# Li-Qingyun/RSCoTr

Measured on AMD Instinct MI355X. Metric: images/sec MTL train step (Swin-T 512^2, bs=2/GPU), higher is better.
Workload: dtype f32 (large products as three fp16 MFMAs on two-plane power-of-two-scaled splits of the fp32 operands, fp32 accumulate: fp32-FMA-class error; six bf16 MFMAs on three-plane splits where an operand has no range word)

## Files before the change

rscotr_amd/csrc/swin_attn.hip:

```cpp
#include "common.h"
#include "rscotr.h"

namespace rscotr {

constexpr int WS = 7, WN = 49, HD = 32, TBL = 169;
constexpr int WATTN_PBIAS = 172, WATTN_PROW = WATTN_PBIAS + 3 * HD;

struct WinGeom {
  int H, W, Hp, Wp, nWw, nW, C, heads, shift;
};

struct TokPos {
  bool pad;
  long tok;
  int label;
};

__device__ __forceinline__ TokPos win_token(const WinGeom& g, int wy, int wx, int t) {
  TokPos r;
  const int ys = wy * WS + t / WS, xs = wx * WS + t % WS;
  int yo = ys + g.shift, xo = xs + g.shift;
  if (yo >= g.Hp) yo -= g.Hp;
  if (xo >= g.Wp) xo -= g.Wp;
  r.pad = (yo >= g.H) || (xo >= g.W);
  r.tok = (long)yo * g.W + xo;
  const int ry = ys < g.Hp - WS ? 0 : (ys < g.Hp - g.shift ? 1 : 2);
  const int rx = xs < g.Wp - WS ? 0 : (xs < g.Wp - g.shift ? 1 : 2);
  r.label = ry * 3 + rx;
  return r;
}

constexpr int LDT = HD + 1;
constexpr int NPD = WN + 1;
constexpr int LDP = NPD + 1;

typedef float f32x16 __attribute__((ext_vector_type(16)));

struct TileRegs {
  float4 v[(WN * (HD / 4) + 63) / 64];
};

__device__ __forceinline__ void tile_load(TileRegs& r, const float* __restrict__ src_tok0, long tok_stride,
                                          const float* __restrict__ pad_vals, const int* sTok, int lane) {
#pragma unroll
  for (int i = 0; i < 7; ++i) {
    const int idx = lane + i * 64;
    r.v[i] = make_float4(0.f, 0.f, 0.f, 0.f);
    if (idx < WN * (HD / 4)) {
      const int t = idx >> 3, c4 = idx & 7;
      const int tok = sTok[t];
      if (tok >= 0) r.v[i] = *reinterpret_cast<const float4*>(src_tok0 + (long)tok * tok_stride + c4 * 4);
      else if (pad_vals) r.v[i] = *reinterpret_cast<const float4*>(pad_vals + c4 * 4);
    }
  }
}

__device__ __forceinline__ void tile_store(const TileRegs& r, float* dst, float scale, int lane) {
#pragma unroll
  for (int i = 0; i < 7; ++i) {
    const int idx = lane + i * 64;
    if (idx < WN * (HD / 4)) {
      float* d = dst + (idx >> 3) * LDT + (idx & 7) * 4;
      d[0] = r.v[i].x * scale; d[1] = r.v[i].y * scale; d[2] = r.v[i].z * scale; d[3] = r.v[i].w * scale;
    }
  }
}

__device__ __forceinline__ void zero16(f32x16& a) {
#pragma unroll
  for (int r = 0; r < 16; ++r) a[r] = 0.f;
}

__device__ __forceinline__ int crow(int r, int lane) { return (r & 3) + 8 * (r >> 2) + 4 * (lane >> 5); }

__device__ __forceinline__ float half_sum(float v) {
#pragma unroll
  for (int o = 16; o > 0; o >>= 1) v += __shfl_xor(v, o, 64);
  return v;
}

__device__ __forceinline__ void mma_rr1(f32x16& acc, const float* A, const float* B, int mi, int ni, int lane) {
  const int fr = lane & 31, fk = lane >> 5;
  const float* a = A + min(mi * 32 + fr, WN - 1) * LDT + fk;
  const float* b = B + min(ni * 32 + fr, WN - 1) * LDT + fk;
#pragma unroll
  for (int kk = 0; kk < HD; kk += 2) acc = __builtin_amdgcn_mfma_f32_32x32x2f32(a[kk], b[kk], acc, 0, 0, 0);
}

__device__ __forceinline__ void mma_pt1(f32x16& acc, const float* SP, const float* T, int mi, int lane) {
  const int fr = lane & 31, fk = lane >> 5;
  const float* a = SP + min(mi * 32 + fr, WN) * LDP + fk;
#pragma unroll 5
  for (int kk = 0; kk < NPD; kk += 2)
    acc = __builtin_amdgcn_mfma_f32_32x32x2f32(a[kk], T[min(kk + fk, WN - 1) * LDT + fr], acc, 0, 0, 0);
}

__device__ __forceinline__ void mma_ptT1(f32x16& acc, const float* SP, const float* T, int mi, int lane) {
  const int fr = lane & 31, fk = lane >> 5;
  const int j = min(mi * 32 + fr, WN);
#pragma unroll 5
  for (int kk = 0; kk < NPD; kk += 2)
    acc = __builtin_amdgcn_mfma_f32_32x32x2f32(SP[(kk + fk) * LDP + j], T[min(kk + fk, WN - 1) * LDT + fr], acc, 0, 0, 0);
}

__device__ __forceinline__ void store_scores1(const f32x16& acc, float* sP, const float* sT, const int* sLab, int shift,
                                              int mi, int ni, int lane) {
  const int fr = lane & 31;
  const int j = ni * 32 + fr, jc = min(j, WN - 1);
  const int jb = (6 - jc / WS) * 13 + (6 - jc % WS), jl = sLab[jc];
#pragma unroll
  for (int r = 0; r < 16; ++r) {
    const int i = mi * 32 + crow(r, lane);
    if (i >= WN || j >= WN) continue;
    const int ti = (i / WS) * 13 + i % WS;
    sP[i * LDP + j] = acc[r] + sT[ti + jb] + ((shift > 0 && jl != sLab[i]) ? -100.0f : 0.f);
  }
}

__device__ __forceinline__ void softmax_rows4(float* sP, int tid) {
  const int row = tid >> 2, q = tid & 3;
  float* rowp = sP + min(row, WN - 1) * LDP;
  float v[13];
  float m = -3.0e38f;
#pragma unroll
  for (int u = 0; u < 13; ++u) {
    const int j = q + 4 * u;
    v[u] = j < WN ? rowp[j] : -3.0e38f;
    m = fmaxf(m, v[u]);
  }
  m = fmaxf(m, __shfl_xor(m, 1, 64));
  m = fmaxf(m, __shfl_xor(m, 2, 64));
  float sum = 0.f;
#pragma unroll
  for (int u = 0; u < 13; ++u) {
    v[u] = (q + 4 * u < WN) ? __expf(v[u] - m) : 0.f;
    sum += v[u];
  }
  sum += __shfl_xor(sum, 1, 64);
  sum += __shfl_xor(sum, 2, 64);
  const float inv = 1.f / sum;
  if (row < WN) {
#pragma unroll
    for (int u = 0; u < 13; ++u)
      if (q + 4 * u < WN) rowp[q + 4 * u] = v[u] * inv;
  }
}

__device__ __forceinline__ void stage_item_tiles(float* sQ, float* sK, float* sV, float* sG, const float* base,
                                                 const float* __restrict__ qkv_b, const float* dout_b, const WinGeom& g,
                                                 int head, const int* sTok, float scale, int w, int lane) {
  if (w == 3 && !dout_b) return;
  const float* src = w == 3 ? dout_b : base + w * g.C;
  const long tstride = w == 3 ? g.C : 3 * g.C;
  const float* padv = (w == 3 || !qkv_b) ? nullptr : qkv_b + w * g.C + head * HD;
  float* dst = w == 0 ? sQ : (w == 1 ? sK : (w == 2 ? sV : sG));
  TileRegs r;
  tile_load(r, src, tstride, padv, sTok, lane);
  tile_store(r, dst, w == 0 ? scale : 1.f, lane);
}

__global__ __launch_bounds__(256) void swin_wattn_fwd_mfma4_kernel(const float* __restrict__ qkv,
                                                                   const float* __restrict__ qkv_b,
                                                                   const float* __restrict__ table,
                                                                   float* __restrict__ out, WinGeom g, int B,
                                                                   unsigned* __restrict__ amax_out) {
  __shared__ float sQ[WN * LDT], sK[WN * LDT], sV[WN * LDT];
  __shared__ float sP[NPD * LDP];
  __shared__ float sT[TBL];
  __shared__ int sLab[WN], sTok[WN];
  float amx = 0.f;
  const int tid = threadIdx.x, lane = tid & 63, w = tid >> 6;
  const int head = blockIdx.x % g.heads;
  const int stride = gridDim.x / g.heads;
  const float scale = 0.17677669529663687f;
  const long L = (long)g.H * g.W;
  for (int t = tid; t < TBL; t += 256) sT[t] = table[t * g.heads + head];
  for (int t = tid; t < NPD * LDP; t += 256) sP[t] = 0.f;
  for (int bw = blockIdx.x / g.heads; bw < B * g.nW; bw += stride) {
    const int b = bw / g.nW, win = bw % g.nW, wy = win / g.nWw, wx = win % g.nWw;
    __syncthreads();
    if (tid < WN) {
      const TokPos me = win_token(g, wy, wx, tid);
      sLab[tid] = me.label;
      sTok[tid] = me.pad ? -1 : (int)me.tok;
    }
    __syncthreads();
    stage_item_tiles(sQ, sK, sV, nullptr, qkv + (long)b * L * 3 * g.C + head * HD, qkv_b, nullptr, g, head, sTok, scale, w, lane);
    __syncthreads();
    {
      f32x16 a;
      zero16(a);
      mma_rr1(a, sQ, sK, w >> 1, w & 1, lane);
      store_scores1(a, sP, sT, sLab, g.shift, w >> 1, w & 1, lane);
    }
    __syncthreads();
    softmax_rows4(sP, tid);
    __syncthreads();
    if (w < 2) {
      f32x16 o;
      zero16(o);
      mma_pt1(o, sP, sV, w, lane);
#pragma unroll
      for (int r = 0; r < 16; ++r) {
        const int i = w * 32 + crow(r, lane);
        if (i < WN) {
          const int tok = sTok[i];
          if (tok >= 0) { out[((long)b * L + tok) * g.C + head * HD + (lane & 31)] = o[r]; amx = fmaxf(amx, fabsf(o[r])); }
        }
      }
    }
  }
  amax_commit(amax_out, amx);
}

__device__ __forceinline__ void swin_wattn_bwd_mfma4_body(const float* __restrict__ qkv,
                                                                   const float* __restrict__ qkv_b,
                                                                   const float* __restrict__ table,
                                                                   const float* __restrict__ dout,
                                                                   const float* __restrict__ outp,
                                                                   float* __restrict__ dqkv, float* __restrict__ part,
                                                                   const WinGeom& g, int B, unsigned* __restrict__ amax_out) {
  __shared__ float sQ[WN * LDT], sK[WN * LDT], sV[WN * LDT], sG[WN * LDT];
  __shared__ float sP[NPD * LDP];
  __shared__ float sT[TBL];
  __shared__ float sBw[4][3 * HD];
  float amx = 0.f;
  __shared__ float sDelta[64];
  __shared__ int sLab[WN], sTok[WN];
  const int tid = threadIdx.x, lane = tid & 63, w = tid >> 6, fr = lane & 31;
  const int head = blockIdx.x % g.heads;
  const int stride = gridDim.x / g.heads;
  const float scale = 0.17677669529663687f;
  const long L = (long)g.H * g.W;
  for (int t = tid; t < TBL; t += 256) sT[t] = table[t * g.heads + head];
  for (int t = tid; t < NPD * LDP; t += 256) sP[t] = 0.f;
  float dT = 0.f;
  float accB[3] = {0.f, 0.f, 0.f};
  const int tdy = tid / 13 - 6, tdx = tid % 13 - 6;
  const int iy0 = max(0, tdy), iy1 = min(6, 6 + tdy), ix0 = max(0, tdx), ix1 = min(6, 6 + tdx);
  for (int bw = blockIdx.x / g.heads; bw < B * g.nW; bw += stride) {
    const int b = bw / g.nW, win = bw % g.nW, wy = win / g.nWw, wx = win % g.nWw;
    __syncthreads();
    if (tid < WN) {
      const TokPos me = win_token(g, wy, wx, tid);
      sLab[tid] = me.label;
      sTok[tid] = me.pad ? -1 : (int)me.tok;
    }
    __syncthreads();
    float4 o_a = make_float4(0.f, 0.f, 0.f, 0.f), o_b = o_a;
    if (outp && (tid >> 2) < WN) {
      const int tok = sTok[tid >> 2];
      if (tok >= 0) {
        const float4* o4 = reinterpret_cast<const float4*>(outp + ((long)b * L + tok) * g.C + head * HD + (tid & 3) * 8);
        o_a = o4[0];
        o_b = o4[1];
      }
    }
    stage_item_tiles(sQ, sK, sV, sG, qkv + (long)b * L * 3 * g.C + head * HD, qkv_b, dout + (long)b * L * g.C + head * HD, g,
                     head, sTok, scale, w, lane);
    __syncthreads();
    float* dq_base = dqkv + (long)b * L * 3 * g.C + head * HD;
    if (outp) {
      const float* gq = sG + min(tid >> 2, WN - 1) * LDT + (tid & 3) * 8;
      float d = ((o_a.x * gq[0] + o_a.y * gq[1]) + (o_a.z * gq[2] + o_a.w * gq[3])) +
                ((o_b.x * gq[4] + o_b.y * gq[5]) + (o_b.z * gq[6] + o_b.w * gq[7]));
      d += __shfl_xor(d, 1, 64);
      d += __shfl_xor(d, 2, 64);
      if ((tid & 3) == 0) sDelta[tid >> 2] = d;
    }
    {
      f32x16 a;
      zero16(a);
      mma_rr1(a, sQ, sK, w >> 1, w & 1, lane);
      store_scores1(a, sP, sT, sLab, g.shift, w >> 1, w & 1, lane);
    }
    __syncthreads();
    softmax_rows4(sP, tid);
    __syncthreads();
    f32x16 dp[2];
    if (w < 2) {
      zero16(dp[0]); zero16(dp[1]);
      mma_rr1(dp[0], sG, sV, w, 0, lane);
      mma_rr1(dp[1], sG, sV, w, 1, lane);
    } else {
      f32x16 dv;
      zero16(dv);
      mma_ptT1(dv, sP, sG, w - 2, lane);
#pragma unroll
      for (int r = 0; r < 16; ++r) {
        const int j = (w - 2) * 32 + crow(r, lane);
        if (j < WN) {
          const int tok = sTok[j];
          if (tok >= 0) { dq_base[(long)tok * 3 * g.C + 2 * g.C + fr] = dv[r]; amx = fmaxf(amx, fabsf(dv[r])); }
          else accB[2] += dv[r];
        }
      }
    }
    __syncthreads();
    if (w < 2) {
#pragma unroll
      for (int r = 0; r < 16; ++r) {
        const int i = w * 32 + crow(r, lane);
        const bool iv = i < WN;
        const int j0 = fr, j1 = 32 + fr;
        const float p0 = iv ? sP[i * LDP + j0] : 0.f;
        const float p1 = (iv && j1 < WN) ? sP[i * LDP + j1] : 0.f;
        const float delta = outp ? sDelta[min(i, 63)] : half_sum(p0 * dp[0][r] + p1 * dp[1][r]);
        if (iv) {
          sP[i * LDP + j0] = p0 * (dp[0][r] - delta);
          if (j1 < WN) sP[i * LDP + j1] = p1 * (dp[1][r] - delta);
        }
      }
    }
    __syncthreads();
    if (w < 2) {
      f32x16 dq;
      zero16(dq);
      mma_pt1(dq, sP, sK, w, lane);
#pragma unroll
      for (int r = 0; r < 16; ++r) {
        const int i = w * 32 + crow(r, lane);
        if (i < WN) {
          const int tok = sTok[i];
          if (tok >= 0) { dq_base[(long)tok * 3 * g.C + fr] = dq[r] * scale; amx = fmaxf(amx, fabsf(dq[r] * scale)); }
          else accB[0] += dq[r] * scale;
        }
      }
    } else {
      f32x16 dk;
      zero16(dk);
      mma_ptT1(dk, sP, sQ, w - 2, lane);
#pragma unroll
      for (int r = 0; r < 16; ++r) {
        const int j = (w - 2) * 32 + crow(r, lane);
        if (j < WN) {
          const int tok = sTok[j];
          if (tok >= 0) { dq_base[(long)tok * 3 * g.C + g.C + fr] = dk[r]; amx = fmaxf(amx, fabsf(dk[r])); }
          else accB[1] += dk[r];
        }
      }
    }
    if (tid < TBL) {
      float acc7 = 0.f;
#pragma unroll 1
      for (int iy = iy0; iy <= iy1; ++iy) {
        float v[WS];
#pragma unroll
        for (int ix = 0; ix < WS; ++ix) {
          const bool ok = ix >= ix0 && ix <= ix1;
          v[ix] = ok ? sP[(iy * WS + ix) * LDP + (iy - tdy) * WS + (ix - tdx)] : 0.f;
        }
        acc7 += ((v[0] + v[1]) + (v[2] + v[3])) + ((v[4] + v[5]) + v[6]);
      }
      dT += acc7;
    }
  }
#pragma unroll
  for (int k = 0; k < 3; ++k) {
    const float other = __shfl_xor(accB[k], 32, 64);
    if (lane < 32) sBw[w][k * HD + fr] = accB[k] + other;
  }
  __syncthreads();
  float* prow = part + (long)blockIdx.x * WATTN_PROW;
  if (tid < TBL) prow[tid] = dT;
  if (tid < 3 * HD) prow[WATTN_PBIAS + tid] = ((sBw[0][tid] + sBw[1][tid]) + sBw[2][tid]) + sBw[3][tid];
  amax_commit(amax_out, amx);
}

template <int OCC>
__global__ __launch_bounds__(256) __attribute__((amdgpu_waves_per_eu(OCC, OCC))) void swin_wattn_bwd_mfma4_kernel(
    const float* __restrict__ qkv, const float* __restrict__ qkv_b, const float* __restrict__ table,
    const float* __restrict__ dout, const float* __restrict__ outp, float* __restrict__ dqkv, float* __restrict__ part,
    WinGeom g, int B, unsigned* __restrict__ amax_out) {
  swin_wattn_bwd_mfma4_body(qkv, qkv_b, table, dout, outp, dqkv, part, g, B, amax_out);
}

static int wattn_geom(const char* fn, WinGeom* g, int B, int H, int W, int C, int heads, int ws, int shift) {
  if (B < 0 || H <= 0 || W <= 0 || C <= 0 || heads <= 0)
    return fail(RSCOTR_E_SHAPE, "%s: bad shape B=%d H=%d W=%d C=%d heads=%d", fn, B, H, W, C, heads);
  if (ws != WS) return fail(RSCOTR_E_SHAPE, "%s: window size %d (only 7 is built)", fn, ws);
  if (C != heads * HD) return fail(RSCOTR_E_SHAPE, "%s: C=%d must be heads*32 (heads=%d)", fn, C, heads);
  if (shift < 0 || shift >= WS) return fail(RSCOTR_E_SHAPE, "%s: shift %d outside [0,7)", fn, shift);
  g->H = H; g->W = W; g->C = C; g->heads = heads; g->shift = shift;
  g->Hp = (H + WS - 1) / WS * WS;
  g->Wp = (W + WS - 1) / WS * WS;
  g->nWw = g->Wp / WS;
  g->nW = (g->Hp / WS) * g->nWw;
  return RSCOTR_OK;
}

static int wattn_grid(const WinGeom& g, int B, int per_cu) {
  const long items = (long)B * g.nW;
  long per_head = std::min<long>(items, std::max<long>(1, (256L * per_cu) / g.heads));
  return (int)(per_head * g.heads);
}

}

using namespace rscotr;

extern "C" int rscotr_swin_wattn_fwd(const float* qkv, const float* qkv_bias, const float* bias_table,
                                     float* out, int B, int H, int W, int C, int heads, int ws, int shift,
                                     uint32_t* amax_out, void* stream) {
  WinGeom g;
  if (int e = wattn_geom("rscotr_swin_wattn_fwd", &g, B, H, W, C, heads, ws, shift)) return e;
  if (B == 0) return RSCOTR_OK;
  if (!qkv || !bias_table || !out) return fail(RSCOTR_E_ARG, "rscotr_swin_wattn_fwd: null pointer");
  if (!aligned16(qkv) || !aligned16(out) || (qkv_bias && !aligned16(qkv_bias)))
    return fail(RSCOTR_E_ALIGN, "rscotr_swin_wattn_fwd: pointers must be 16-byte aligned");
  const double items = (double)B * ((H + ws - 1) / ws) * ((W + ws - 1) / ws) * heads;
  ProfScope prof(PROF_MFMA, items * 4.0 * 49 * 49 * 32, (hipStream_t)stream, "rscotr::swin_wattn_fwd_kernel");
  swin_wattn_fwd_mfma4_kernel<<<wattn_grid(g, B, 4), 256, 0, (hipStream_t)stream>>>(qkv, qkv_bias, bias_table, out, g, B, amax_out);
  return check_launch("rscotr_swin_wattn_fwd");
}

static int wattn_bwd_grid(const WinGeom& g, int B) { return wattn_grid(g, B, 4); }

namespace rscotr {
__global__ __launch_bounds__(256) void wattn_param_fold_kernel(const float* __restrict__ part, float* __restrict__ dtable,
                                                               float* __restrict__ dqkv_b, int heads, int C, int rows) {
  __shared__ float red[3][64];
  const int lane = threadIdx.x & 63, w = threadIdx.x >> 6;
  const int col = blockIdx.x * 64 + lane, head = blockIdx.y;
  float a = 0.f;
  if (col < WATTN_PROW) {
#pragma unroll 8
    for (int r = w; r < rows; r += 4) a += part[((long)r * heads + head) * WATTN_PROW + col];
  }
  if (w > 0) red[w - 1][lane] = a;
  __syncthreads();
  if (w != 0 || col >= WATTN_PROW) return;
  a += red[0][lane];
  a += red[1][lane];
  a += red[2][lane];
  if (col < TBL) {
    if (dtable) dtable[col * heads + head] += a;
  } else if (col >= WATTN_PBIAS && dqkv_b) {
    const int t = col - WATTN_PBIAS;
    dqkv_b[(t / HD) * C + head * HD + (t % HD)] += a;
  }
}

__global__ __launch_bounds__(256) void wattn_param_flush_kernel(const int64_t* __restrict__ table, int n) {
  __shared__ float red[3][64];
  int e = 0;
  while (e + 1 < n && (int)table[(long)(e + 1) * 16 + 6] <= (int)blockIdx.y) ++e;
  const int64_t* t = table + (long)e * 16;
  const float* part = reinterpret_cast<const float*>(t[0]);
  float* dtable = reinterpret_cast<float*>(t[1]);
  float* dqkv_b = reinterpret_cast<float*>(t[2]);
  const int heads = (int)t[3], C = (int)t[4], rows = (int)t[5], head = (int)blockIdx.y - (int)t[6];
  const int lane = threadIdx.x & 63, w = threadIdx.x >> 6;
  const int col = blockIdx.x * 64 + lane;
  float a = 0.f;
  if (col < WATTN_PROW) {
#pragma unroll 8
    for (int r = w; r < rows; r += 4) a += part[((long)r * heads + head) * WATTN_PROW + col];
  }
  if (w > 0) red[w - 1][lane] = a;
  __syncthreads();
  if (w != 0 || col >= WATTN_PROW) return;
  a += red[0][lane];
  a += red[1][lane];
  a += red[2][lane];
  if (col < TBL) {
    if (dtable) dtable[col * heads + head] += a;
  } else if (col >= WATTN_PBIAS && dqkv_b) {
    const int c = col - WATTN_PBIAS;
    dqkv_b[(c / HD) * C + head * HD + (c % HD)] += a;
  }
}
}

extern "C" int rscotr_swin_wattn_flush(const int64_t* table, int n, int total_heads, void* stream) {
  if (n < 0 || total_heads < 0) return fail(RSCOTR_E_SHAPE, "rscotr_swin_wattn_flush: negative count");
  if (n == 0 || total_heads == 0) return RSCOTR_OK;
  if (!table) return fail(RSCOTR_E_ARG, "rscotr_swin_wattn_flush: null table");
  wattn_param_flush_kernel<<<dim3((WATTN_PROW + 63) / 64, (unsigned)total_heads), 256, 0, (hipStream_t)stream>>>(table, n);
  return check_launch("rscotr_swin_wattn_flush");
}

extern "C" int64_t rscotr_swin_wattn_bwd_workspace(int B, int H, int W, int C, int heads) {
  WinGeom g;
  if (B <= 0 || wattn_geom("rscotr_swin_wattn_bwd_workspace", &g, B, H, W, C, heads, WS, 0)) return 0;
  return (int64_t)wattn_bwd_grid(g, B) * WATTN_PROW * 4;
}

extern "C" int rscotr_swin_wattn_bwd(const float* qkv, const float* qkv_bias, const float* bias_table,
                                     const float* dout, float* dqkv, float* dqkv_bias, float* dbias_table,
                                     int B, int H, int W, int C, int heads, int ws, int shift, const float* out,
                                     float* workspace, int64_t workspace_bytes, uint32_t* amax_out, void* stream) {
  WinGeom g;
  if (int e = wattn_geom("rscotr_swin_wattn_bwd", &g, B, H, W, C, heads, ws, shift)) return e;
  if (B == 0) return RSCOTR_OK;
  if (!qkv || !bias_table || !dout || !dqkv) return fail(RSCOTR_E_ARG, "rscotr_swin_wattn_bwd: null pointer");
  if (!aligned16(qkv) || !aligned16(dout) || !aligned16(dqkv) || (qkv_bias && !aligned16(qkv_bias)))
    return fail(RSCOTR_E_ALIGN, "rscotr_swin_wattn_bwd: pointers must be 16-byte aligned");
  const int nwg = wattn_bwd_grid(g, B);
  if (!workspace || workspace_bytes < (int64_t)nwg * WATTN_PROW * 4)
    return fail(RSCOTR_E_ARG, "rscotr_swin_wattn_bwd: workspace of rscotr_swin_wattn_bwd_workspace() bytes required");
  hipStream_t s = (hipStream_t)stream;
  const double items = (double)B * ((H + ws - 1) / ws) * ((W + ws - 1) / ws) * heads;
  ProfScope prof(PROF_MFMA, items * 10.0 * 49 * 49 * 32, s, "rscotr::swin_wattn_bwd_kernel");
  const float* o = (out && aligned16(out)) ? out : nullptr;
  if (nwg > 512 && nwg <= 768) swin_wattn_bwd_mfma4_kernel<3><<<nwg, 256, 0, s>>>(qkv, qkv_bias, bias_table, dout, o, dqkv, workspace, g, B, amax_out);
  else swin_wattn_bwd_mfma4_kernel<2><<<nwg, 256, 0, s>>>(qkv, qkv_bias, bias_table, dout, o, dqkv, workspace, g, B, amax_out);
  if (dbias_table || dqkv_bias)
    wattn_param_fold_kernel<<<dim3((WATTN_PROW + 63) / 64, heads), 256, 0, s>>>(workspace, dbias_table, dqkv_bias, heads, C,
                                                                              nwg / heads);
  return check_launch("rscotr_swin_wattn_bwd");
}
```

Before: 204.3.

## Prefetch next window's tiles into registers and pack row metadata words

The Swin window-attention forward and backward kernels now double-buffer per-window row metadata and issue the global loads for the next window's Q/K/V (and dout/out) tiles into registers while the current window computes. This overlaps global memory latency with the MFMA work. Token offset, pad flag and mask label are packed into one int word, stored in a crow-permuted copy, and read as int4 so the scatter stores drop per-row index math. The forward grid drops from 4 to 3 blocks per CU to offset the added register pressure. Backward prefetch is enabled only for the OCC==2 instantiation, and byte offsets are now 32-bit with a new shape guard.

```diff
diff --git a/rscotr_amd/csrc/swin_attn.hip b/rscotr_amd/csrc/swin_attn.hip
--- a/rscotr_amd/csrc/swin_attn.hip
+++ b/rscotr_amd/csrc/swin_attn.hip
@@ -40,16 +40,51 @@
   float4 v[(WN * (HD / 4) + 63) / 64];
 };
 
-__device__ __forceinline__ void tile_load(TileRegs& r, const float* __restrict__ src_tok0, long tok_stride,
-                                          const float* __restrict__ pad_vals, const int* sTok, int lane) {
+constexpr int ROW_PAD = (int)0x80000000, ROW_NONE = -1;
+
+__device__ __forceinline__ int crow_slot(int i) { return (i & 32) | ((i & 4) << 2) | ((i & 24) >> 1) | (i & 3); }
+
+__device__ __forceinline__ void write_rows(int* sRow, int* sRowC, const WinGeom& g, int bw, int t) {
+  const int win = bw % g.nW, wy = win / g.nWw, wx = win % g.nWw;
+  int word = ROW_NONE;
+  if (t < WN) {
+    const TokPos me = win_token(g, wy, wx, t);
+    word = (me.pad ? ROW_PAD : (int)me.tok * g.C) | me.label;
+  }
+  sRow[t] = word;
+  sRowC[crow_slot(t)] = word;
+}
+
+struct RowWords {
+  int e[16];
+};
+
+__device__ __forceinline__ void load_rows(RowWords& rw, const int* sRowC, int mi, int lane) {
+  const int4* p = reinterpret_cast<const int4*>(sRowC + mi * 32 + (lane >> 5) * 16);
+#pragma unroll
+  for (int q = 0; q < 4; ++q) {
+    const int4 v = p[q];
+    rw.e[4 * q] = v.x; rw.e[4 * q + 1] = v.y; rw.e[4 * q + 2] = v.z; rw.e[4 * q + 3] = v.w;
+  }
+}
+
+__device__ __forceinline__ const float* at_bytes(const float* base, unsigned bytes) {
+  return reinterpret_cast<const float*>(reinterpret_cast<const char*>(base) + bytes);
+}
+__device__ __forceinline__ float* at_bytes(float* base, unsigned bytes) {
+  return reinterpret_cast<float*>(reinterpret_cast<char*>(base) + bytes);
+}
+
+__device__ __forceinline__ void tile_load(TileRegs& r, const float* __restrict__ src_tok0, unsigned mul,
+                                          const float* __restrict__ pad_vals, const int* sRow, int lane) {
 #pragma unroll
   for (int i = 0; i < 7; ++i) {
     const int idx = lane + i * 64;
     r.v[i] = make_float4(0.f, 0.f, 0.f, 0.f);
     if (idx < WN * (HD / 4)) {
       const int t = idx >> 3, c4 = idx & 7;
-      const int tok = sTok[t];
-      if (tok >= 0) r.v[i] = *reinterpret_cast<const float4*>(src_tok0 + (long)tok * tok_stride + c4 * 4);
+      const int e = sRow[t];
+      if (e >= 0) r.v[i] = *reinterpret_cast<const float4*>(at_bytes(src_tok0, (unsigned)(e & ~15) * (4u * mul) + c4 * 16u));
       else if (pad_vals) r.v[i] = *reinterpret_cast<const float4*>(pad_vals + c4 * 4);
     }
   }
@@ -103,17 +138,29 @@
     acc = __builtin_amdgcn_mfma_f32_32x32x2f32(SP[(kk + fk) * LDP + j], T[min(kk + fk, WN - 1) * LDT + fr], acc, 0, 0, 0);
 }
 
-__device__ __forceinline__ void store_scores1(const f32x16& acc, float* sP, const float* sT, const int* sLab, int shift,
-                                              int mi, int ni, int lane) {
+__device__ __forceinline__ void store_scores1(const f32x16& acc, float* sP, const float* sT, const int* sRow,
+                                              const RowWords& rw, int shift, int mi, int ni, int lane) {
   const int fr = lane & 31;
   const int j = ni * 32 + fr, jc = min(j, WN - 1);
-  const int jb = (6 - jc / WS) * 13 + (6 - jc % WS), jl = sLab[jc];
+  const int jb = (6 - jc / WS) * 13 + (6 - jc % WS), jl = sRow[jc] & 15;
+  const int i0 = mi * 32 + 4 * (lane >> 5);
 #pragma unroll
   for (int r = 0; r < 16; ++r) {
-    const int i = mi * 32 + crow(r, lane);
-    if (i >= WN || j >= WN) continue;
-    const int ti = (i / WS) * 13 + i % WS;
-    sP[i * LDP + j] = acc[r] + sT[ti + jb] + ((shift > 0 && jl != sLab[i]) ? -100.0f : 0.f);
+    const int i = i0 + (r & 3) + 8 * (r >> 2), ic = min(i, WN - 1);
+    const float v = acc[r] + sT[(ic / WS) * 13 + ic % WS + jb] + ((shift > 0 && jl != (rw.e[r] & 15)) ? -100.0f : 0.f);
+    if (i < WN && j < WN) sP[i * LDP + j] = v;
+  }
+}
+
+template <unsigned MUL>
+__device__ __forceinline__ void store_rows(const f32x16& acc, const RowWords& rw, float* dst_col, float& padsum, float& amx) {
+#pragma unroll
+  for (int r = 0; r < 16; ++r) {
+    const int e = rw.e[r];
+    const float v = acc[r];
+    if (e >= 0) *at_bytes(dst_col, (unsigned)(e & ~15) * (4u * MUL)) = v;
+    amx = fmaxf(amx, e >= 0 ? fabsf(v) : 0.f);
+    padsum += (e < ROW_NONE) ? v : 0.f;
   }
 }
 
@@ -146,16 +193,19 @@
   }
 }
 
-__device__ __forceinline__ void stage_item_tiles(float* sQ, float* sK, float* sV, float* sG, const float* base,
-                                                 const float* __restrict__ qkv_b, const float* dout_b, const WinGeom& g,
-                                                 int head, const int* sTok, float scale, int w, int lane) {
+__device__ __forceinline__ void item_tile_load(TileRegs& r, const float* qkv_b, const float* __restrict__ qkv_bias,
+                                               const float* dout_b, const WinGeom& g, int head, const int* sRow, int w,
+                                               int lane) {
   if (w == 3 && !dout_b) return;
-  const float* src = w == 3 ? dout_b : base + w * g.C;
-  const long tstride = w == 3 ? g.C : 3 * g.C;
-  const float* padv = (w == 3 || !qkv_b) ? nullptr : qkv_b + w * g.C + head * HD;
+  const float* src = (w == 3 ? dout_b : qkv_b + w * g.C) + head * HD;
+  const float* padv = (w == 3 || !qkv_bias) ? nullptr : qkv_bias + w * g.C + head * HD;
+  tile_load(r, src, w == 3 ? 1u : 3u, padv, sRow, lane);
+}
+
+__device__ __forceinline__ void item_tile_store(const TileRegs& r, float* sQ, float* sK, float* sV, float* sG, float scale,
+                                                int w, int lane) {
+  if (w == 3 && !sG) return;
   float* dst = w == 0 ? sQ : (w == 1 ? sK : (w == 2 ? sV : sG));
-  TileRegs r;
-  tile_load(r, src, tstride, padv, sTok, lane);
   tile_store(r, dst, w == 0 ? scale : 1.f, lane);
 }
 
@@ -167,52 +217,75 @@
   __shared__ float sQ[WN * LDT], sK[WN * LDT], sV[WN * LDT];
   __shared__ float sP[NPD * LDP];
   __shared__ float sT[TBL];
-  __shared__ int sLab[WN], sTok[WN];
+  __shared__ __attribute__((aligned(16))) int sRow[2][64], sRowC[2][64];
   float amx = 0.f;
   const int tid = threadIdx.x, lane = tid & 63, w = tid >> 6;
   const int head = blockIdx.x % g.heads;
-  const int stride = gridDim.x / g.heads;
+  const int stride = gridDim.x / g.heads, nitems = B * g.nW;
   const float scale = 0.17677669529663687f;
   const long L = (long)g.H * g.W;
   for (int t = tid; t < TBL; t += 256) sT[t] = table[t * g.heads + head];
   for (int t = tid; t < NPD * LDP; t += 256) sP[t] = 0.f;
-  for (int bw = blockIdx.x / g.heads; bw < B * g.nW; bw += stride) {
-    const int b = bw / g.nW, win = bw % g.nW, wy = win / g.nWw, wx = win % g.nWw;
-    __syncthreads();
-    if (tid < WN) {
-      const TokPos me = win_token(g, wy, wx, tid);
-      sLab[tid] = me.label;
-      sTok[tid] = me.pad ? -1 : (int)me.tok;
-    }
-    __syncthreads();
-    stage_item_tiles(sQ, sK, sV, nullptr, qkv + (long)b * L * 3 * g.C + head * HD, qkv_b, nullptr, g, head, sTok, scale, w, lane);
-    __syncthreads();
+  int bw = blockIdx.x / g.heads;
+  if (w == 3) write_rows(sRow[0], sRowC[0], g, bw, lane);
+  __syncthreads();
+  TileRegs tr;
+  item_tile_load(tr, qkv + (long)(bw / g.nW) * L * 3 * g.C, qkv_b, nullptr, g, head, sRow[0], w, lane);
+  float unused = 0.f;
+  for (int cur = 0; bw < nitems; bw += stride, cur ^= 1) {
+    const int nxt = bw + stride;
+    __syncthreads();
+    if (w < 3) item_tile_store(tr, sQ, sK, sV, nullptr, scale, w, lane);
+    else if (nxt < nitems) write_rows(sRow[cur ^ 1], sRowC[cur ^ 1], g, nxt, lane);
+    __syncthreads();
+    if (nxt < nitems) item_tile_load(tr, qkv + (long)(nxt / g.nW) * L * 3 * g.C, qkv_b, nullptr, g, head, sRow[cur ^ 1], w, lane);
     {
+      RowWords rw;
+      load_rows(rw, sRowC[cur], w >> 1, lane);
       f32x16 a;
       zero16(a);
       mma_rr1(a, sQ, sK, w >> 1, w & 1, lane);
-      store_scores1(a, sP, sT, sLab, g.shift, w >> 1, w & 1, lane);
+      store_scores1(a, sP, sT, sRow[cur], rw, g.shift, w >> 1, w & 1, lane);
     }
     __syncthreads();
     softmax_rows4(sP, tid);
     __syncthreads();
     if (w < 2) {
+      RowWords rw;
+      load_rows(rw, sRowC[cur], w, lane);
       f32x16 o;
       zero16(o);
       mma_pt1(o, sP, sV, w, lane);
-#pragma unroll
-      for (int r = 0; r < 16; ++r) {
-        const int i = w * 32 + crow(r, lane);
-        if (i < WN) {
-          const int tok = sTok[i];
-          if (tok >= 0) { out[((long)b * L + tok) * g.C + head * HD + (lane & 31)] = o[r]; amx = fmaxf(amx, fabsf(o[r])); }
-        }
-      }
+      store_rows<1>(o, rw, out + (long)(bw / g.nW) * L * g.C + head * HD + (lane & 31), unused, amx);
     }
   }
   amax_commit(amax_out, amx);
 }
 
+struct ItemRegs {
+  TileRegs t;
+  float4 o_a, o_b;
+};
+
+__device__ __forceinline__ void bwd_item_load(ItemRegs& ir, const float* __restrict__ qkv, const float* __restrict__ qkv_b,
+                                              const float* __restrict__ dout, const float* __restrict__ outp,
+                                              const WinGeom& g, long L, int bw, int head, const int* sRow, int tid) {
+  const int b = bw / g.nW, lane = tid & 63, w = tid >> 6;
+  ir.o_a = make_float4(0.f, 0.f, 0.f, 0.f);
+  ir.o_b = ir.o_a;
+  if (outp) {
+    const int e = sRow[tid >> 2];
+    if (e >= 0) {
+      const float4* o4 = reinterpret_cast<const float4*>(
+          at_bytes(outp + (long)b * L * g.C + head * HD, (unsigned)(e & ~15) * 4u + (tid & 3) * 32u));
+      ir.o_a = o4[0];
+      ir.o_b = o4[1];
+    }
+  }
+  item_tile_load(ir.t, qkv + (long)b * L * 3 * g.C, qkv_b, dout + (long)b * L * g.C, g, head, sRow, w, lane);
+}
+
+template <bool PF>
 __device__ __forceinline__ void swin_wattn_bwd_mfma4_body(const float* __restrict__ qkv,
                                                                    const float* __restrict__ qkv_b,
                                                                    const float* __restrict__ table,
@@ -226,10 +299,10 @@
   __shared__ float sBw[4][3 * HD];
   float amx = 0.f;
   __shared__ float sDelta[64];
-  __shared__ int sLab[WN], sTok[WN];
+  __shared__ __attribute__((aligned(16))) int sRow[2][64], sRowC[2][64];
   const int tid = threadIdx.x, lane = tid & 63, w = tid >> 6, fr = lane & 31;
   const int head = blockIdx.x % g.heads;
-  const int stride = gridDim.x / g.heads;
+  const int stride = gridDim.x / g.heads, nitems = B * g.nW;
   const float scale = 0.17677669529663687f;
   const long L = (long)g.H * g.W;
   for (int t = tid; t < TBL; t += 256) sT[t] = table[t * g.heads + head];
@@ -238,28 +311,20 @@
   float accB[3] = {0.f, 0.f, 0.f};
   const int tdy = tid / 13 - 6, tdx = tid % 13 - 6;
   const int iy0 = max(0, tdy), iy1 = min(6, 6 + tdy), ix0 = max(0, tdx), ix1 = min(6, 6 + tdx);
-  for (int bw = blockIdx.x / g.heads; bw < B * g.nW; bw += stride) {
-    const int b = bw / g.nW, win = bw % g.nW, wy = win / g.nWw, wx = win % g.nWw;
-    __syncthreads();
-    if (tid < WN) {
-      const TokPos me = win_token(g, wy, wx, tid);
-      sLab[tid] = me.label;
-      sTok[tid] = me.pad ? -1 : (int)me.tok;
-    }
-    __syncthreads();
-    float4 o_a = make_float4(0.f, 0.f, 0.f, 0.f), o_b = o_a;
-    if (outp && (tid >> 2) < WN) {
-      const int tok = sTok[tid >> 2];
-      if (tok >= 0) {
-        const float4* o4 = reinterpret_cast<const float4*>(outp + ((long)b * L + tok) * g.C + head * HD + (tid & 3) * 8);
-        o_a = o4[0];
-        o_b = o4[1];
-      }
-    }
-    stage_item_tiles(sQ, sK, sV, sG, qkv + (long)b * L * 3 * g.C + head * HD, qkv_b, dout + (long)b * L * g.C + head * HD, g,
-                     head, sTok, scale, w, lane);
-    __syncthreads();
-    float* dq_base = dqkv + (long)b * L * 3 * g.C + head * HD;
+  int bw = blockIdx.x / g.heads;
+  if (w == 3) write_rows(sRow[0], sRowC[0], g, bw, lane);
+  __syncthreads();
+  ItemRegs ir;
+  if (PF) bwd_item_load(ir, qkv, qkv_b, dout, outp, g, L, bw, head, sRow[0], tid);
+  for (int cur = 0; bw < nitems; bw += stride, cur ^= 1) {
+    const int b = bw / g.nW, nxt = bw + stride;
+    if (!PF) bwd_item_load(ir, qkv, qkv_b, dout, outp, g, L, bw, head, sRow[cur], tid);
+    __syncthreads();
+    item_tile_store(ir.t, sQ, sK, sV, sG, scale, w, lane);
+    if (w == 3 && nxt < nitems) write_rows(sRow[cur ^ 1], sRowC[cur ^ 1], g, nxt, lane);
+    __syncthreads();
+    const float4 o_a = ir.o_a, o_b = ir.o_b;
+    float* dq_col = dqkv + (long)b * L * 3 * g.C + head * HD + fr;
     if (outp) {
       const float* gq = sG + min(tid >> 2, WN - 1) * LDT + (tid & 3) * 8;
       float d = ((o_a.x * gq[0] + o_a.y * gq[1]) + (o_a.z * gq[2] + o_a.w * gq[3])) +
@@ -268,11 +333,14 @@
       d += __shfl_xor(d, 2, 64);
       if ((tid & 3) == 0) sDelta[tid >> 2] = d;
     }
+    if (PF && nxt < nitems) bwd_item_load(ir, qkv, qkv_b, dout, outp, g, L, nxt, head, sRow[cur ^ 1], tid);
+    RowWords rw;
     {
+      load_rows(rw, sRowC[cur], w >> 1, lane);
       f32x16 a;
       zero16(a);
       mma_rr1(a, sQ, sK, w >> 1, w & 1, lane);
-      store_scores1(a, sP, sT, sLab, g.shift, w >> 1, w & 1, lane);
+      store_scores1(a, sP, sT, sRow[cur], rw, g.shift, w >> 1, w & 1, lane);
     }
     __syncthreads();
     softmax_rows4(sP, tid);
@@ -286,15 +354,8 @@
       f32x16 dv;
       zero16(dv);
       mma_ptT1(dv, sP, sG, w - 2, lane);
-#pragma unroll
-      for (int r = 0; r < 16; ++r) {
-        const int j = (w - 2) * 32 + crow(r, lane);
-        if (j < WN) {
-          const int tok = sTok[j];
-          if (tok >= 0) { dq_base[(long)tok * 3 * g.C + 2 * g.C + fr] = dv[r]; amx = fmaxf(amx, fabsf(dv[r])); }
-          else accB[2] += dv[r];
-        }
-      }
+      load_rows(rw, sRowC[cur], w & 1, lane);
+      store_rows<3>(dv, rw, dq_col + 2 * g.C, accB[2], amx);
     }
     __syncthreads();
     if (w < 2) {
@@ -313,32 +374,19 @@
       }
     }
     __syncthreads();
+    load_rows(rw, sRowC[cur], w & 1, lane);
     if (w < 2) {
       f32x16 dq;
       zero16(dq);
       mma_pt1(dq, sP, sK, w, lane);
 #pragma unroll
-      for (int r = 0; r < 16; ++r) {
-        const int i = w * 32 + crow(r, lane);
-        if (i < WN) {
-          const int tok = sTok[i];
-          if (tok >= 0) { dq_base[(long)tok * 3 * g.C + fr] = dq[r] * scale; amx = fmaxf(amx, fabsf(dq[r] * scale)); }
-          else accB[0] += dq[r] * scale;
-        }
-      }
+      for (int r = 0; r < 16; ++r) dq[r] = __fmul_rn(dq[r], scale);
+      store_rows<3>(dq, rw, dq_col, accB[0], amx);
     } else {
       f32x16 dk;
       zero16(dk);
       mma_ptT1(dk, sP, sQ, w - 2, lane);
-#pragma unroll
-      for (int r = 0; r < 16; ++r) {
-        const int j = (w - 2) * 32 + crow(r, lane);
-        if (j < WN) {
-          const int tok = sTok[j];
-          if (tok >= 0) { dq_base[(long)tok * 3 * g.C + g.C + fr] = dk[r]; amx = fmaxf(amx, fabsf(dk[r])); }
-          else accB[1] += dk[r];
-        }
-      }
+      store_rows<3>(dk, rw, dq_col + g.C, accB[1], amx);
     }
     if (tid < TBL) {
       float acc7 = 0.f;
@@ -372,7 +420,7 @@
     const float* __restrict__ qkv, const float* __restrict__ qkv_b, const float* __restrict__ table,
     const float* __restrict__ dout, const float* __restrict__ outp, float* __restrict__ dqkv, float* __restrict__ part,
     WinGeom g, int B, unsigned* __restrict__ amax_out) {
-  swin_wattn_bwd_mfma4_body(qkv, qkv_b, table, dout, outp, dqkv, part, g, B, amax_out);
+  swin_wattn_bwd_mfma4_body<OCC == 2>(qkv, qkv_b, table, dout, outp, dqkv, part, g, B, amax_out);
 }
 
 static int wattn_geom(const char* fn, WinGeom* g, int B, int H, int W, int C, int heads, int ws, int shift) {
@@ -381,6 +429,7 @@
   if (ws != WS) return fail(RSCOTR_E_SHAPE, "%s: window size %d (only 7 is built)", fn, ws);
   if (C != heads * HD) return fail(RSCOTR_E_SHAPE, "%s: C=%d must be heads*32 (heads=%d)", fn, C, heads);
   if (shift < 0 || shift >= WS) return fail(RSCOTR_E_SHAPE, "%s: shift %d outside [0,7)", fn, shift);
+  if ((long)H * W * C * 12 > 0xFFFFFFFFL) return fail(RSCOTR_E_SHAPE, "%s: H*W*C=%ld: an image's qkv slice exceeds 4 GB", fn, (long)H * W * C);
   g->H = H; g->W = W; g->C = C; g->heads = heads; g->shift = shift;
   g->Hp = (H + WS - 1) / WS * WS;
   g->Wp = (W + WS - 1) / WS * WS;
@@ -410,7 +459,7 @@
     return fail(RSCOTR_E_ALIGN, "rscotr_swin_wattn_fwd: pointers must be 16-byte aligned");
   const double items = (double)B * ((H + ws - 1) / ws) * ((W + ws - 1) / ws) * heads;
   ProfScope prof(PROF_MFMA, items * 4.0 * 49 * 49 * 32, (hipStream_t)stream, "rscotr::swin_wattn_fwd_kernel");
-  swin_wattn_fwd_mfma4_kernel<<<wattn_grid(g, B, 4), 256, 0, (hipStream_t)stream>>>(qkv, qkv_bias, bias_table, out, g, B, amax_out);
+  swin_wattn_fwd_mfma4_kernel<<<wattn_grid(g, B, 3), 256, 0, (hipStream_t)stream>>>(qkv, qkv_bias, bias_table, out, g, B, amax_out);
   return check_launch("rscotr_swin_wattn_fwd");
 }
 
```

Result: no change. 205.2, median of 6 (+0.4%).
